# facebookresearch/audiocraft

Hardware: NVIDIA B200
Metric: MusicGen-medium audio-sec/sec @30s gen (higher is better)
Workload: dtype f16

## Files before the change

audiocraft_b200/csrc/lm.cu:

```cuda
#include "common.cuh"
#include "lm_step.cuh"
#include <math.h>
#include <new>
#include <vector>
#include <algorithm>
#include <utility>
#include <stdio.h>
#include <stdlib.h>

__device__ __forceinline__ void mma16816(float (&c)[4], uint32_t a0, uint32_t a1, uint32_t a2, uint32_t a3, uint32_t b0,
                                         uint32_t b1) {
    asm volatile(
        "mma.sync.aligned.m16n8k16.row.col.f32.f16.f16.f32 {%0,%1,%2,%3}, {%4,%5,%6,%7}, {%8,%9}, {%0,%1,%2,%3};"
        : "+f"(c[0]), "+f"(c[1]), "+f"(c[2]), "+f"(c[3])
        : "r"(a0), "r"(a1), "r"(a2), "r"(a3), "r"(b0), "r"(b1));
}

__device__ __forceinline__ void pdl_trigger() { asm volatile("griddepcontrol.launch_dependents;" ::: "memory"); }
__device__ __forceinline__ void pdl_wait() { asm volatile("griddepcontrol.wait;" ::: "memory"); }

#ifdef ACB_TIMELINE
__device__ __forceinline__ void tl_stamp(unsigned long long* t, int slot) {
    if (t && threadIdx.x == 0) {
        unsigned long long now;
// ... 104 lines not shown
    tl_stamp(timing, 5);
    float q = 0.f;
    if (live) {
        const float cx = a.x - mean, cy = a.y - mean, cz = a.z - mean, cw = a.w - mean;
        q = fmaf(cx, cx, q); q = fmaf(cy, cy, q); q = fmaf(cz, cz, q); q = fmaf(cw, cw, q);
    }
    const float rstd = 1.f / sqrtf(block_sum(q, red[1]) / d + 1e-5f);
    tl_stamp(timing, 6);
    if (live) {
        __half2 lo = __floats2half2_rn((a.x - mean) * rstd * gm.x + bt.x, (a.y - mean) * rstd * gm.y + bt.y);
        __half2 hi = __floats2half2_rn((a.z - mean) * rstd * gm.z + bt.z, (a.w - mean) * rstd * gm.w + bt.w);
        uint2 pk;
        pk.x = *reinterpret_cast<uint32_t*>(&lo);
        pk.y = *reinterpret_cast<uint32_t*>(&hi);
        reinterpret_cast<uint2*>(out + (size_t)r * d)[i] = pk;
    }
    tl_stamp(timing, 3);
}

enum { EPI_PARTIAL = 0, EPI_QKV = 1, EPI_GELU = 2, EPI_F32 = 3, EPI_CROSSKV = 4, EPI_QKV_PF = 5 };

struct GemmParams {
    const __half* W;
    const __half* X;
    int N, K, rows, kslice;
    float* out_f32; int ld_out; size_t split_stride;
    __half* out_f16;
    float* q32; __half* kc; __half* vc; int d, H, cache_len; const int* pos;
    int text_len, row0;
    int rows_real;
    unsigned long long* timing;
};

template <int NT, int EPI, int FT2 = 1>
__global__ void __launch_bounds__(128) lm_gemm_kernel(GemmParams p) {
#ifndef ACB_GEMM_U2
#define ACB_GEMM_U2 4
#endif
    constexpr int U = NT <= 2 ? ACB_GEMM_U2 : (NT <= 4 ? 2 : 1);
    constexpr int RP = 8 * NT + 1;
    constexpr int FB = 16 * FT2;
    extern __shared__ __align__(128) unsigned char gsm[];
    const int tid = threadIdx.x, warp = tid >> 5, lane = tid & 31, g = lane >> 2, c4 = lane & 3;
    const int f0 = blockIdx.x * FB;
    const int k0 = blockIdx.y * p.kslice;
    const int ks = min(p.kslice, p.K - k0);
    const int pitch = p.kslice * 2 + 64;
    uint64_t* bar = reinterpret_cast<uint64_t*>(gsm + FB * pitch);
    float* red = reinterpret_cast<float*>(gsm + FB * pitch + 16);

    tl_stamp(p.timing, 0);
    if (tid == 0) mbar_init(bar, 1);
    __syncthreads();
    if (tid == 0) {
        mbar_expect_tx(bar, (uint32_t)FB * (uint32_t)ks * 2u);
#pragma unroll 1
        for (int r = 0; r < FB; ++r)
            bulk_g2s(gsm + r * pitch, p.W + (size_t)(f0 + r) * p.K + k0, (uint32_t)ks * 2u, bar);
    }
    pdl_trigger();
    pdl_wait();
    tl_stamp(p.timing, 1);
    int cache_pos = 0;
    if (EPI == EPI_QKV || EPI == EPI_QKV_PF) cache_pos = p.pos[0];

    float c[FT2][NT][4];
#pragma unroll
    for (int ft = 0; ft < FT2; ++ft)
#pragma unroll
        for (int j = 0; j < NT; ++j) c[ft][j][0] = c[ft][j][1] = c[ft][j][2] = c[ft][j][3] = 0.f;

    const int nkb = ks >> 5;
    const int kbw = (nkb + 3) >> 2;
    const int kb0 = min(nkb, warp * kbw), kb1 = min(nkb, kb0 + kbw);
    const __half* xr = p.X + (size_t)g * p.K + k0 + 8 * c4;
    const unsigned char* wr0 = gsm + g * pitch + 16 * c4;
    const unsigned char* wr1 = wr0 + 8 * pitch;

    bool w_ready = false;
    for (int kb = kb0; kb < kb1; kb += U) {
        uint4 xv[U][NT];
#pragma unroll
        for (int u = 0; u < U; ++u)
#pragma unroll
            for (int j = 0; j < NT; ++j)
                xv[u][j] = (kb + u < kb1) ? *reinterpret_cast<const uint4*>(xr + (size_t)(8 * j) * p.K + (size_t)(kb + u) * 32)
                                          : make_uint4(0, 0, 0, 0);
        if (!w_ready) { mbar_wait(bar, 0); w_ready = true; tl_stamp(p.timing, 4); }
#pragma unroll
        for (int u = 0; u < U; ++u) {
            if (kb + u < kb1) {
#pragma unroll
                for (int ft = 0; ft < FT2; ++ft) {
                    const uint4 wa = *reinterpret_cast<const uint4*>(wr0 + ft * 16 * pitch + (kb + u) * 64);
                    const uint4 wb = *reinterpret_cast<const uint4*>(wr1 + ft * 16 * pitch + (kb + u) * 64);
#pragma unroll
                    for (int j = 0; j < NT; ++j) {
                        mma16816(c[ft][j], wa.x, wb.x, wa.y, wb.y, xv[u][j].x, xv[u][j].y);
                        mma16816(c[ft][j], wa.z, wb.z, wa.w, wb.w, xv[u][j].z, xv[u][j].w);
                    }
                }
            }
        }
    }
    if (!w_ready) mbar_wait(bar, 0);
    tl_stamp(p.timing, 2);
#pragma unroll
    for (int ft = 0; ft < FT2; ++ft)
#pragma unroll
        for (int j = 0; j < NT; ++j) {
            float* r0 = red + (warp * FB + ft * 16 + g) * RP + 8 * j + 2 * c4;
            r0[0] = c[ft][j][0];
            r0[1] = c[ft][j][1];
// ... 184 lines not shown
        }
        __threadfence();
        __syncthreads();
        if (tid == 0) is_last = atomicAdd(p.counter + row * p.H + h, 1) == nact - 1;
        __syncthreads();
        if (is_last) {
            __threadfence();
            if (tid < 64) {
                float M = -INFINITY;
                for (int z = 0; z < nact; ++z) M = fmaxf(M, __ldcg(rec + z * 66));
                float L = 0.f, O = 0.f;
                for (int z = 0; z < nact; ++z) {
                    const float cz = __expf(__ldcg(rec + z * 66) - M);
                    L = fmaf(__ldcg(rec + z * 66 + 1), cz, L);
                    O = fmaf(__ldcg(rec + z * 66 + 2 + tid), cz, O);
                }
                p.out[(size_t)row * p.d + h * 64 + tid] = __float2half_rn(O / L);
            }
            if (tid == 0) p.counter[row * p.H + h] = 0;
        }
    }
    tl_stamp(p.timing, 3);
}

constexpr int ATT2_DEPTH = 8;
__global__ void __launch_bounds__(ATT_WARPS * 32) lm_attn2_kernel(AttnParams p) {
    extern __shared__ __align__(16) unsigned char att2sm[];
    __shared__ float wm[ATT_WARPS], wl[ATT_WARPS], wacc[ATT_WARPS][64];
    const int h = blockIdx.x, tid = threadIdx.x, warp = tid >> 5, lane = tid & 31;
    const int row = blockIdx.y;
    const int sl = lane & 7, pg = lane >> 3;
    tl_stamp(p.timing, 0);
    pdl_trigger();
    pdl_wait();
    tl_stamp(p.timing, 1);
    const int n = p.fixed_len > 0 ? p.fixed_len : p.pos[0] + 1;
    const size_t base = ((size_t)row * p.H + h) * p.cache_len * 64 + sl * 8;
    const __half* kb = p.kc + base;
    const __half* vb = p.vc + base;
    const uint32_t ring = smem_u32(att2sm) + (uint32_t)(warp * ATT2_DEPTH * 1024 + lane * 16);
    const int n_it = (n + 31 - warp * 4) / 32 > 0 ? (n - warp * 4 + 31) / 32 : 0;
    auto issue = [&](int k) {
        if (k < n_it) {
            const int pp = (k * ATT_WARPS + warp) * 4 + pg;
            if (pp < n) {
                const uint32_t d = ring + (uint32_t)((k % ATT2_DEPTH) * 1024);
                asm volatile("cp.async.cg.shared.global [%0], [%1], 16;" ::"r"(d), "l"(kb + (size_t)pp * 64) : "memory");
                asm volatile("cp.async.cg.shared.global [%0], [%1], 16;" ::"r"(d + 512u), "l"(vb + (size_t)pp * 64) : "memory");
            }
        }
        asm volatile("cp.async.commit_group;" ::: "memory");
    };
#pragma unroll
    for (int k = 0; k < ATT2_DEPTH - 1; ++k) issue(k);

    float q[8];
    {
        const float4* qp = reinterpret_cast<const float4*>(p.q + (size_t)row * p.d + h * 64 + sl * 8);
        const float4 qa = qp[0], qb = qp[1];
        q[0] = half_round(qa.x) * p.scale; q[1] = half_round(qa.y) * p.scale; q[2] = half_round(qa.z) * p.scale;
        q[3] = half_round(qa.w) * p.scale; q[4] = half_round(qb.x) * p.scale; q[5] = half_round(qb.y) * p.scale;
        q[6] = half_round(qb.z) * p.scale; q[7] = half_round(qb.w) * p.scale;
    }
    tl_stamp(p.timing, 4);
    OnlineSM st;
    st.m = -INFINITY; st.l = 0.f;
#pragma unroll
    for (int e = 0; e < 8; ++e) st.acc[e] = 0.f;

    for (int k = 0; k < n_it; ++k) {
        issue(k + ATT2_DEPTH - 1);
        asm volatile("cp.async.wait_group %0;" ::"n"(ATT2_DEPTH - 1) : "memory");
        const int pp = (k * ATT_WARPS + warp) * 4 + pg;
        const uint32_t sa = ring + (uint32_t)((k % ATT2_DEPTH) * 1024);
        uint4 kv = make_uint4(0, 0, 0, 0), vv = make_uint4(0, 0, 0, 0);
        if (pp < n) {
            asm volatile("ld.shared.v4.u32 {%0,%1,%2,%3}, [%4];" : "=r"(kv.x), "=r"(kv.y), "=r"(kv.z), "=r"(kv.w) : "r"(sa));
            asm volatile("ld.shared.v4.u32 {%0,%1,%2,%3}, [%4];" : "=r"(vv.x), "=r"(vv.y), "=r"(vv.z), "=r"(vv.w) : "r"(sa + 512u));
        }
        const __half2* k2 = reinterpret_cast<const __half2*>(&kv);
        float s = 0.f;
#pragma unroll
        for (int e = 0; e < 4; ++e) {
            const float2 f = __half22float2(k2[e]);
            s = fmaf(q[2 * e], f.x, s);
            s = fmaf(q[2 * e + 1], f.y, s);
        }
        s += __shfl_xor_sync(0xffffffffu, s, 1);
        s += __shfl_xor_sync(0xffffffffu, s, 2);
        s += __shfl_xor_sync(0xffffffffu, s, 4);
        if (pp < n) {
            const float mn = fmaxf(st.m, s);
            const float corr = __expf(st.m - mn);
            const float pw = __expf(s - mn);
            st.l = st.l * corr + pw;
            const __half2* v2 = reinterpret_cast<const __half2*>(&vv);
#pragma unroll
            for (int e = 0; e < 4; ++e) {
                const float2 f = __half22float2(v2[e]);
                st.acc[2 * e] = fmaf(pw, f.x, st.acc[2 * e] * corr);
                st.acc[2 * e + 1] = fmaf(pw, f.y, st.acc[2 * e + 1] * corr);
            }
            st.m = mn;
        }
// ... 5 lines not shown
        const float m2 = __shfl_xor_sync(0xffffffffu, st.m, o), l2 = __shfl_xor_sync(0xffffffffu, st.l, o);
        float a2[8];
#pragma unroll
        for (int e = 0; e < 8; ++e) a2[e] = __shfl_xor_sync(0xffffffffu, st.acc[e], o);
        osm_merge(st, m2, l2, a2);
    }
    if (pg == 0) {
        if (sl == 0) { wm[warp] = st.m; wl[warp] = st.l; }
#pragma unroll
        for (int e = 0; e < 8; ++e) wacc[warp][sl * 8 + e] = st.acc[e];
    }
    __syncthreads();
    if (tid < 64) {
        float mx = wm[0];
#pragma unroll
        for (int w = 1; w < ATT_WARPS; ++w) mx = fmaxf(mx, wm[w]);
        float l = 0.f, o = 0.f;
#pragma unroll
        for (int w = 0; w < ATT_WARPS; ++w) {
            const float cw = wm[w] == -INFINITY ? 0.f : __expf(wm[w] - mx);
            l = fmaf(wl[w], cw, l);
            o = fmaf(wacc[w][tid], cw, o);
        }
        p.out[(size_t)row * p.d + h * 64 + tid] = __float2half_rn(o / l);
    }
    tl_stamp(p.timing, 3);
}

template <bool PF>
__global__ void __launch_bounds__(256) lm_cross_attn_kernel(AttnParams p, int rows) {
    __shared__ float qs[8][64];
    const int warp = threadIdx.x >> 5, lane = threadIdx.x & 31;
    const int pair = blockIdx.x * 8 + warp;
    tl_stamp(p.timing, 0);
    pdl_trigger();
    pdl_wait();
    tl_stamp(p.timing, 1);
    if (pair >= rows * p.H) return;
    const int row = pair / p.H, h = pair % p.H, n = p.fixed_len;
    {
        const float* qp = p.q + (size_t)row * p.d + h * 64 + lane * 2;
        float2 part[ACB_LM_MAX_SPLIT];
#pragma unroll
        for (int s = 0; s < ACB_LM_MAX_SPLIT; ++s)
            part[s] = s < p.q_nsplit ? *reinterpret_cast<const float2*>(qp + s * p.q_split_stride) : make_float2(0.f, 0.f);
        float a0 = 0.f, a1 = 0.f;
#pragma unroll
        for (int s = 0; s < ACB_LM_MAX_SPLIT; ++s) { a0 += part[s].x; a1 += part[s].y; }
        qs[warp][lane * 2] = half_round(a0) * p.scale;
        qs[warp][lane * 2 + 1] = half_round(a1) * p.scale;
    }
    __syncwarp();
    tl_stamp(p.timing, 4);
    const size_t base = ((size_t)(PF ? row % p.rows_real : row) * p.H + h) * p.cache_len * 64;
    float mx = -INFINITY, l = 0.f, o0 = 0.f, o1 = 0.f;
    for (int t0 = 0; t0 < n; t0 += 32) {
        const int t = t0 + lane;
        float s = -INFINITY;
        if (t < n) {
            const uint4* kr = reinterpret_cast<const uint4*>(p.kc + base + (size_t)t * 64);
            s = 0.f;
#pragma unroll
            for (int c = 0; c < 8; ++c) {
                const uint4 kk = kr[c];
                const __half2* k2 = reinterpret_cast<const __half2*>(&kk);
#pragma unroll
                for (int e = 0; e < 4; ++e) {
                    const float2 f = __half22float2(k2[e]);
                    s = fmaf(qs[warp][c * 8 + 2 * e], f.x, s);
                    s = fmaf(qs[warp][c * 8 + 2 * e + 1], f.y, s);
                }
            }
        }
        tl_stamp(p.timing, 5);
        const float cm = fmaxf(mx, warp_max(s));
        const float corr = mx == -INFINITY ? 0.f : __expf(mx - cm);
        const float pw = t < n ? __expf(s - cm) : 0.f;
        l = l * corr + warp_sum(pw);
        o0 *= corr; o1 *= corr;
        tl_stamp(p.timing, 6);
        const int cnt = min(32, n - t0);
        for (int j = 0; j < cnt; ++j) {
            const float wj = __shfl_sync(0xffffffffu, pw, j);
            const float2 f = __half22float2(*reinterpret_cast<const __half2*>(p.vc + base + (size_t)(t0 + j) * 64 + lane * 2));
            o0 = fmaf(wj, f.x, o0);
            o1 = fmaf(wj, f.y, o1);
        }
        mx = cm;
    }
    tl_stamp(p.timing, 2);
    *reinterpret_cast<__half2*>(p.out + (size_t)row * p.d + h * 64 + lane * 2) = __floats2half2_rn(o0 / l, o1 / l);
    tl_stamp(p.timing, 3);
}

__device__ __forceinline__ uint4 philox4x32_10(uint4 ctr, uint2 key) {
    const uint32_t M0 = 0xD2511F53u, M1 = 0xCD9E8D57u, W0 = 0x9E3779B9u, W1 = 0xBB67AE85u;
#pragma unroll
    for (int r = 0; r < 10; ++r) {
        uint32_t hi0 = __umulhi(M0, ctr.x), lo0 = M0 * ctr.x;
        uint32_t hi1 = __umulhi(M1, ctr.z), lo1 = M1 * ctr.z;
        ctr = make_uint4(hi1 ^ ctr.y ^ key.x, lo1, hi0 ^ ctr.w ^ key.y, lo0);
        key.x += W0;
        key.y += W1;
    }
    return ctr;
}
__device__ __forceinline__ float exp1_noise(uint64_t seed, uint32_t step, uint32_t stream, uint32_t i) {
    uint4 r = philox4x32_10(make_uint4(i >> 2, stream, step, 0x5a17u), make_uint2((uint32_t)seed, (uint32_t)(seed >> 32)));
    uint32_t w = (i & 3) == 0 ? r.x : ((i & 3) == 1 ? r.y : ((i & 3) == 2 ? r.z : r.w));
    float u = ((float)(w >> 8) + 0.5f) * (1.0f / 16777216.0f);
    return -logf(u);
}

struct SampleParams {
    const float* logits;
    const float* noise;
    float* logits_out;
    int64_t* seq; const uint8_t* seq_mask; int* pos; int max_seq;
    int64_t* tokens;
// ... 146 lines not shown
    if (tid == 0) {
        for (int w = 1; w < (nt >> 5); ++w)
            if (bestv[w] > bv || (bestv[w] == bv && besti[w] < bi)) { bv = bestv[w]; bi = besti[w]; }
        if (bi == 0x7fffffff) bi = 0;
        int tok = sorted_space ? si[bi] : bi;
        if (p.tokens) p.tokens[(size_t)b * p.n_q + k] = tok;
        if (p.seq) {
            const int off = cur_pos + 1;
            if (off < p.max_seq) {
                if (!p.seq_mask[(size_t)k * p.max_seq + off]) tok = card;
                int64_t* dst = p.seq + ((size_t)b * p.n_q + k) * p.max_seq + off;
                if (*dst == -1) *dst = tok;
            }
            __threadfence();
            const int done = atomicAdd(p.pos + 1, 1);
            if (done == (int)(gridDim.x * gridDim.y) - 1) { p.pos[1] = 0; p.pos[0] = cur_pos + 1; }
        }
    }
}

__global__ void lm_f32_to_f16_kernel(const float* __restrict__ src, __half* __restrict__ dst, size_t n_valid, size_t n_total) {
    size_t i = (size_t)blockIdx.x * blockDim.x + threadIdx.x;
    if (i < n_total) dst[i] = __float2half_rn(i < n_valid ? src[i] : 0.f);
}

struct acb_lm {
    acb_lm_config cfg;
    acb_lm_weights w;
    acb_lm_buffers buf;
    acb_lm_sampling samp;
    cudaStream_t capture_stream = nullptr;
    cudaGraph_t graph = nullptr;
    cudaGraphExec_t exec = nullptr;
    int batch = 0, rows = 0, rows_pad = 0, text_len = 0, seq_len = 0, sms = 148;
    int launches = 0;
    bool has_cross = false;
    bool pdl = true;
    bool attn2 = true;
    bool fused = false;
    StepLaunch step{};
    unsigned long long* trace = nullptr;
    unsigned long long* timing = nullptr;
    struct TimedGemm { const char* what; int ctas; };
    std::vector<TimedGemm> timed;
};
constexpr int ACB_TIMING_MAX_CTAS = 1024, ACB_TIMING_MAX_GEMMS = 16;
constexpr size_t ACB_PLAN_COUNTER_BYTES = 4096;

template <typename... KArgs, typename... Args>
static cudaError_t launch_k(void (*kernel)(KArgs...), dim3 grid, dim3 block, size_t smem, cudaStream_t s, bool pdl,
                            Args... args) {
    cudaLaunchConfig_t cfg{};
    cfg.gridDim = grid; cfg.blockDim = block; cfg.dynamicSmemBytes = smem; cfg.stream = s;
    cudaLaunchAttribute attr[1];
    if (pdl) {
        attr[0].id = cudaLaunchAttributeProgrammaticStreamSerialization;
        attr[0].val.programmaticStreamSerializationAllowed = 1;
        cfg.attrs = attr; cfg.numAttrs = 1;
    }
    return cudaLaunchKernelEx(&cfg, kernel, KArgs(args)...);
}
#define ACB_LAUNCH(...) ACB_CHECK_CUDA(launch_k(__VA_ARGS__))

static int nt_for_rows(int rows) { return rows <= 8 ? 1 : (rows <= 16 ? 2 : (rows <= 32 ? 4 : 8)); }

static size_t gemm_smem_bytes(int nt, int kslice, int ft2 = 1) {
    return (size_t)16 * ft2 * (kslice * 2 + 64) + 16 + (size_t)4 * 16 * ft2 * (8 * nt + 1) * sizeof(float);
}
constexpr int GEMM_MAX_SMEM = 120 * 1024;

template <int EPI, int FT2>
static int launch_gemm_ft(int nt, const GemmParams& p, int nsplit, cudaStream_t s, bool pdl) {
    dim3 grid(p.N / (16 * FT2), nsplit);
    const size_t smem = gemm_smem_bytes(nt, p.kslice, FT2);
    ACB_REQUIRE(smem <= (size_t)GEMM_MAX_SMEM && p.N % (16 * FT2) == 0, "lm_gemm: tile does not fit (N=%d kslice=%d ft2=%d)", p.N, p.kslice, FT2);
    switch (nt) {
        case 1: ACB_LAUNCH((lm_gemm_kernel<1, EPI, FT2>), grid, dim3(128), smem, s, pdl, p); break;
        case 2: ACB_LAUNCH((lm_gemm_kernel<2, EPI, FT2>), grid, dim3(128), smem, s, pdl, p); break;
        case 4: ACB_LAUNCH((lm_gemm_kernel<4, EPI, FT2>), grid, dim3(128), smem, s, pdl, p); break;
        default: ACB_LAUNCH((lm_gemm_kernel<8, EPI, FT2>), grid, dim3(128), smem, s, pdl, p); break;
    }
    return ACB_OK;
}
template <int EPI>
static int launch_gemm(int nt, const GemmParams& p, int nsplit, cudaStream_t s, bool pdl, int ft2 = 1) {
    if (ft2 == 2) {
        if constexpr (EPI == EPI_CROSSKV || EPI == EPI_QKV_PF) { acb_set_error("lm_gemm: this epilogue uses 16-feature tiles"); return ACB_ERR_INVALID; }
        else return launch_gemm_ft<EPI, 2>(nt, p, nsplit, s, pdl);
    }
    return launch_gemm_ft<EPI, 1>(nt, p, nsplit, s, pdl);
}

template <int NT, int EPI, int FT2>
static cudaError_t gemm_attr_one() {
    cudaError_t e = cudaFuncSetAttribute(lm_gemm_kernel<NT, EPI, FT2>, cudaFuncAttributeMaxDynamicSharedMemorySize, GEMM_MAX_SMEM);
    if (e != cudaSuccess) return e;
    return cudaFuncSetAttribute(lm_gemm_kernel<NT, EPI, FT2>, cudaFuncAttributePreferredSharedMemoryCarveout, 100);
}
template <int EPI>
static cudaError_t gemm_attr_all() {
    cudaError_t e;
    if ((e = gemm_attr_one<1, EPI, 1>()) != cudaSuccess) return e;
    if ((e = gemm_attr_one<2, EPI, 1>()) != cudaSuccess) return e;
    if ((e = gemm_attr_one<4, EPI, 1>()) != cudaSuccess) return e;
    if ((e = gemm_attr_one<8, EPI, 1>()) != cudaSuccess) return e;
    if constexpr (EPI != EPI_CROSSKV && EPI != EPI_QKV_PF) {
        if ((e = gemm_attr_one<1, EPI, 2>()) != cudaSuccess) return e;
        if ((e = gemm_attr_one<2, EPI, 2>()) != cudaSuccess) return e;
        if ((e = gemm_attr_one<4, EPI, 2>()) != cudaSuccess) return e;
        if ((e = gemm_attr_one<8, EPI, 2>()) != cudaSuccess) return e;
    }
    return cudaSuccess;
}

static int pick_ft2(int N, int K, int nsplit, int kslice, int nt, int sms) {
    const char* e = getenv("ACB_LM_FT32");
    const bool enabled = !(e && e[0] == '0');
    if (!enabled || N % 32 != 0 || (size_t)N * K < ((size_t)2 << 20)) return 1;
    if ((N / 32) * nsplit * 10 < sms * 9) return 1;
    if (gemm_smem_bytes(nt, kslice, 2) > (size_t)GEMM_MAX_SMEM) return 1;
    return 2;
}

static int pick_split(int N, int K, int sms, bool allow_split, int* kslice) {
    const int nkb = K / 32, tiles = N / 16;
    int ns = 1;
    if (allow_split) {
        ns = max(acb_ceil_div(K, 1536), acb_ceil_div(2 * sms, tiles));
        ns = max(1, min(min(ns, ACB_LM_MAX_SPLIT), nkb / 2 > 0 ? nkb / 2 : 1));
    }
    int kbs = acb_ceil_div(nkb, ns);
    ns = acb_ceil_div(nkb, kbs);
    *kslice = kbs * 32;
    return ns;
}

static GemmParams base_gemm(const void* W, const void* X, int N, int K, int rows, int kslice) {
    GemmParams p{};
    p.W = (const __half*)W;
    p.X = (const __half*)X;
    p.N = N; p.K = K; p.rows = rows; p.kslice = kslice;
    return p;
}

static int env_int(const char* name, int dflt) {
    const char* e = getenv(name);
    return (e && e[0]) ? atoi(e) : dflt;
}

#define ACB_TRY(expr) do { int rc_ = (expr); if (rc_ != ACB_OK) return rc_; } while (0)

static bool acb_debug_on() {
    static int v = -1;
    if (v < 0) { const char* e = getenv("ACB_DEBUG"); v = (e && e[0] == '1') ? 1 : 0; }
    return v == 1;
}
static int acb_dbg(cudaStream_t s, bool capturing, const char* what, int layer) {
    if (!acb_debug_on() || capturing) return ACB_OK;
    fprintf(stderr, "[acb] %s layer %d ... ", what, layer); fflush(stderr);
    cudaError_t e = cudaStreamSynchronize(s);
    fprintf(stderr, "%s\n", cudaGetErrorString(e)); fflush(stderr);
    if (e != cudaSuccess) { acb_set_error("%s (layer %d): %s", what, layer, cudaGetErrorString(e)); return ACB_ERR_CUDA; }
    return ACB_OK;
}
#define DBG(what, layer) ACB_TRY(acb_dbg(s, capturing, what, layer))

static int enqueue_step_kernels(acb_lm* lm, cudaStream_t s, float* logits_out, int* n_launch, bool gemms_only,
                                bool capturing, int pf_tokens = 0) {
    const acb_lm_config& c = lm->cfg;
    const acb_lm_buffers& B = lm->buf;
    const bool pf = pf_tokens > 0;
    const int rows_real = lm->rows, rows = pf ? rows_real * pf_tokens : rows_real;
    const int d = c.dim, ffn = c.ffn_dim, L = c.num_layers, H = c.num_heads, nt = nt_for_rows(rows);
    const size_t part_stride = (size_t)(pf ? 8 * nt : lm->rows_pad) * d;
    const size_t kv_layer = (size_t)c.max_rows * H * c.max_seq * 64;
    const size_t ckv_layer = (size_t)c.max_rows * H * c.max_text * 64;
    const float scale = 1.0f / sqrtf(64.f);
    const bool pdl = lm->pdl;
    int nl = 0, ks = 0;

    if (!gemms_only) {
        if (pf) ACB_LAUNCH(lm_embed_kernel<true>, dim3(rows), dim3(256), 0, s, pdl, (const __half*)lm->w.emb, lm->w.inv_freq,
                           (const int64_t*)B.seq, (const int*)B.pos, B.x, d, c.n_q, c.card, c.max_seq, lm->batch, c.pos_scale, rows_real);
        else ACB_LAUNCH(lm_embed_kernel<false>, dim3(rows), dim3(256), 0, s, pdl, (const __half*)lm->w.emb, lm->w.inv_freq,
                        (const int64_t*)B.seq, (const int*)B.pos, B.x, d, c.n_q, c.card, c.max_seq, lm->batch, c.pos_scale, rows);
        ++nl;
        DBG("lm_embed_kernel", -1);
    }
    enum { G_QKV, G_O, G_CQ, G_CO, G_FF1, G_FF2, G_HEADS };
    int att_split = env_int("ACB_LM_ATT_SPLIT", 1);
    if (att_split < 1 || att_split > 8 || !B.plan ||
        ACB_PLAN_COUNTER_BYTES + (size_t)rows * H * att_split * 66 * sizeof(float) > ACB_LM_PLAN_BYTES ||
        (size_t)rows * H * sizeof(int) > ACB_PLAN_COUNTER_BYTES)
        att_split = 1;
    if (lm->timing && !capturing) lm->timed.clear();
    auto tl = [&](const char* what, int layer, int ctas) -> unsigned long long* {
        if (!lm->timing || capturing || gemms_only || layer != 0 || (int)lm->timed.size() >= ACB_TIMING_MAX_GEMMS ||
            ctas > ACB_TIMING_MAX_CTAS)
            return nullptr;
        unsigned long long* t = lm->timing + (size_t)lm->timed.size() * ACB_TIMING_MAX_CTAS * 8;
        lm->timed.push_back({what, ctas});
        return t;
    };
    int pending = 0;
    auto ln_launch = [&](const float* gamma, const float* beta, int layer) -> int {
        if (gemms_only) return ACB_OK;
        ACB_LAUNCH(lm_ln_kernel, dim3(rows), dim3(LN_THREADS), 0, s, pdl, B.x, (const float*)B.part, pending, part_stride, gamma, beta,
                   (__half*)B.h16, d, tl("ln", layer, rows));
        ++nl;
        DBG("lm_ln_kernel", layer);
        return ACB_OK;
    };
    auto partial_gemm = [&](const __half* W, const void* X, int N, int K, int layer, int id) -> int {
        const int ns = pick_split(N, K, lm->sms, true, &ks);
        GemmParams p = base_gemm(W, X, N, K, rows, ks);
        p.out_f32 = B.part; p.ld_out = N; p.split_stride = part_stride;
        const int ft2 = pick_ft2(N, K, ns, ks, nt, lm->sms);
        p.timing = tl(id == G_O ? "gemm_O" : (id == G_CQ ? "gemm_CQ" : (id == G_CO ? "gemm_CO" : "gemm_FFN2")), layer, (N / (16 * ft2)) * ns);
        ACB_TRY(launch_gemm<EPI_PARTIAL>(nt, p, ns, s, pdl, ft2));
        ++nl;
        DBG("gemm_EPI_PARTIAL", layer);
        pending = ns;
        return ACB_OK;
    };
    for (int l = 0; l < L; ++l) {
        const float* ln = lm->w.ln + (size_t)l * 6 * d;
        ACB_TRY(ln_launch(ln, ln + d, l));
        {
            pick_split(3 * d, d, lm->sms, false, &ks);
            GemmParams p = base_gemm((const __half*)lm->w.w_qkv + (size_t)l * 3 * d * d, B.h16, 3 * d, d, rows, ks);
            p.q32 = B.q32; p.kc = (__half*)B.k_cache + l * kv_layer; p.vc = (__half*)B.v_cache + l * kv_layer;
            p.d = d; p.H = H; p.cache_len = c.max_seq; p.pos = B.pos; p.rows_real = rows_real;
            const int ft2 = pf ? 1 : pick_ft2(3 * d, d, 1, ks, nt, lm->sms);
            p.timing = tl("gemm_QKV", l, 3 * d / (16 * ft2));
            if (pf) ACB_TRY(launch_gemm<EPI_QKV_PF>(nt, p, 1, s, pdl, 1));
            else ACB_TRY(launch_gemm<EPI_QKV>(nt, p, 1, s, pdl, ft2));
            ++nl;
            DBG("gemm_EPI_QKV", l);
        }
        if (!gemms_only) {
            AttnParams a{B.q32, 1, 0, (__half*)B.k_cache + l * kv_layer, (__half*)B.v_cache + l * kv_layer, (__half*)B.a16,
                         H, d, c.max_seq, B.pos, 0, scale};
            a.timing = tl("attn", l, H * rows * att_split);
            a.part = reinterpret_cast<float*>((unsigned char*)B.plan + ACB_PLAN_COUNTER_BYTES);
            a.counter = reinterpret_cast<int*>(B.plan);
            a.split_min = max(129, env_int("ACB_LM_ATT_SPLIT_MIN", 768));
            a.rows_real = rows_real;
            if (pf) ACB_LAUNCH((lm_attn_kernel<false, true>), dim3(H, rows), dim3(ATT_WARPS * 32), 0, s, pdl, a);
            else if (att_split <= 1 && lm->attn2)
                ACB_LAUNCH(lm_attn2_kernel, dim3(H, rows), dim3(ATT_WARPS * 32), (size_t)ATT_WARPS * ATT2_DEPTH * 1024, s, pdl, a);
            else if (att_split > 1) ACB_LAUNCH(lm_attn_kernel<true>, dim3(H, rows, att_split), dim3(ATT_WARPS * 32), 0, s, pdl, a);
            else ACB_LAUNCH(lm_attn_kernel<false>, dim3(H, rows), dim3(ATT_WARPS * 32), 0, s, pdl, a);
            ++nl;
            DBG("lm_attn_kernel", l);
        }
        ACB_TRY(partial_gemm((const __half*)lm->w.w_o + (size_t)l * d * d, B.a16, d, d, l, G_O));
        if (lm->has_cross) {
            ACB_TRY(ln_launch(ln + 2 * d, ln + 3 * d, l));
            ACB_TRY(partial_gemm((const __half*)lm->w.w_cq + (size_t)l * d * d, B.h16, d, d, l, G_CQ));
            const int nsq = pending;
            pending = 0;
            if (!gemms_only) {
                AttnParams a{B.part, nsq, part_stride, (__half*)B.ck_cache + l * ckv_layer,
                             (__half*)B.cv_cache + l * ckv_layer, (__half*)B.a16, H, d, c.max_text, B.pos, lm->text_len,
                             scale};
                a.timing = tl("cross_attn", l, acb_ceil_div(rows * H, 8));
                a.rows_real = rows_real;
                if (pf) ACB_LAUNCH(lm_cross_attn_kernel<true>, dim3(acb_ceil_div(rows * H, 8)), dim3(256), 0, s, pdl, a, rows);
                else ACB_LAUNCH(lm_cross_attn_kernel<false>, dim3(acb_ceil_div(rows * H, 8)), dim3(256), 0, s, pdl, a, rows);
                ++nl;
                DBG("lm_cross_attn_kernel", l);
            }
            ACB_TRY(partial_gemm((const __half*)lm->w.w_co + (size_t)l * d * d, B.a16, d, d, l, G_CO));
        }
        ACB_TRY(ln_launch(ln + 4 * d, ln + 5 * d, l));
        {
            pick_split(ffn, d, lm->sms, false, &ks);
            GemmParams p = base_gemm((const __half*)lm->w.w_ff1 + (size_t)l * ffn * d, B.h16, ffn, d, rows, ks);
            p.out_f16 = (__half*)B.f16; p.ld_out = ffn;
            const int ft2 = pick_ft2(ffn, d, 1, ks, nt, lm->sms);
            p.timing = tl("gemm_FFN1", l, ffn / (16 * ft2));
            ACB_TRY(launch_gemm<EPI_GELU>(nt, p, 1, s, pdl, ft2)); ++nl;
            DBG("gemm_EPI_GELU", l);
        }
        ACB_TRY(partial_gemm((const __half*)lm->w.w_ff2 + (size_t)l * d * ffn, B.f16, d, ffn, l, G_FF2));
    }
    if (pf) {
        if (n_launch) *n_launch = nl;
        return ACB_OK;
    }
    ACB_TRY(ln_launch(lm->w.out_norm, lm->w.out_norm + d, -1));
    {
        const int N = c.n_q * c.card;
        pick_split(N, d, lm->sms, false, &ks);
        GemmParams p = base_gemm(lm->w.heads, B.h16, N, d, rows, ks);
        p.out_f32 = B.logits; p.ld_out = N;
        ACB_TRY(launch_gemm<EPI_F32>(nt, p, 1, s, pdl, pick_ft2(N, d, 1, ks, nt, lm->sms))); ++nl;
        DBG("gemm_EPI_F32", -1);
    }
    if (!gemms_only) {
        int NP = 1;
        while (NP < c.card) NP <<= 1;
        SampleParams sp{B.logits, lm->samp.noise_from_buffer ? B.noise : nullptr, logits_out, B.seq, B.seq_mask, B.pos,
                        c.max_seq, nullptr, lm->batch, rows, c.n_q, c.card, NP, lm->samp.use_sampling, lm->samp.top_k,
                        lm->samp.temp, lm->samp.top_p, lm->samp.cfg_coef, lm->samp.seed, 0, lm->samp.cfg_coef_beta};
        size_t smem = ((size_t)c.card + 2 * (size_t)NP) * sizeof(float);
        ACB_LAUNCH(lm_sample_kernel, dim3(c.n_q, lm->batch), dim3(1024), smem, s, pdl, sp);
        ++nl;
        DBG("lm_sample_kernel", -1);
    }
    if (n_launch) *n_launch = nl;
    return ACB_OK;
}

static int enqueue_step_fused(acb_lm* lm, cudaStream_t s, float* logits_out, int* n_launch, bool step_only, bool capturing) {
    const acb_lm_config& c = lm->cfg;
    const acb_lm_buffers& B = lm->buf;
    int nl = 0;
    ACB_TRY(lm_step_launch(lm->step, s));
    ++nl;
    DBG("lm_step_kernel", -1);
    if (!step_only) {
        int NP = 1;
        while (NP < c.card) NP <<= 1;
        SampleParams sp{B.logits, lm->samp.noise_from_buffer ? B.noise : nullptr, logits_out, B.seq, B.seq_mask, B.pos,
                        c.max_seq, nullptr, lm->batch, lm->rows, c.n_q, c.card, NP, lm->samp.use_sampling, lm->samp.top_k,
                        lm->samp.temp, lm->samp.top_p, lm->samp.cfg_coef, lm->samp.seed, 0, lm->samp.cfg_coef_beta};
        size_t smem = ((size_t)c.card + 2 * (size_t)NP) * sizeof(float);
        ACB_LAUNCH(lm_sample_kernel, dim3(c.n_q, lm->batch), dim3(1024), smem, s, false, sp);
        ++nl;
        DBG("lm_sample_kernel", -1);
    }
    if (n_launch) *n_launch = nl;
    return ACB_OK;
}

static int enqueue_step(acb_lm* lm, cudaStream_t s, float* logits_out, int* n_launch, bool gemms_only = false,
                        bool capturing = false) {
    if (lm->fused) return enqueue_step_fused(lm, s, logits_out, n_launch, gemms_only, capturing);
    return enqueue_step_kernels(lm, s, logits_out, n_launch, gemms_only, capturing);
}

extern "C" int acb_lm_create(const acb_lm_config* cfg, const acb_lm_weights* w, const acb_lm_buffers* buf, acb_lm_t** out) {
    ACB_REQUIRE(cfg && w && buf && out, "acb_lm_create: null argument");
    ACB_REQUIRE(cfg->dim % 64 == 0 && cfg->dim == cfg->num_heads * 64, "acb_lm_create: head_dim must be 64 (dim=%d heads=%d)",
                cfg->dim, cfg->num_heads);
    ACB_REQUIRE(cfg->dim <= 4 * LN_THREADS, "acb_lm_create: dim %d too large for the LayerNorm kernel", cfg->dim);
    ACB_REQUIRE(cfg->ffn_dim % 32 == 0 && cfg->card % 16 == 0 && cfg->n_q >= 1 && cfg->n_q <= 16, "acb_lm_create: bad ffn/card/n_q");
    ACB_REQUIRE(cfg->card <= 4096, "acb_lm_create: card %d > 4096 not built", cfg->card);
    ACB_REQUIRE(cfg->max_rows >= 1 && cfg->max_rows <= 64, "acb_lm_create: max_rows %d not in [1,64]", cfg->max_rows);
    ACB_REQUIRE(cfg->max_seq >= 2 && cfg->max_seq <= 12000, "acb_lm_create: max_seq %d out of range", cfg->max_seq);
    ACB_REQUIRE(cfg->dim <= 2048, "acb_lm_create: dim %d > 2048: the GEMM stages a 16 x dim weight slab per CTA", cfg->dim);
    acb_lm* lm = new (std::nothrow) acb_lm();
    ACB_REQUIRE(lm, "acb_lm_create: out of host memory");
    lm->cfg = *cfg; lm->w = *w; lm->buf = *buf;
    int dev = 0;
    cudaGetDevice(&dev);
    cudaDeviceGetAttribute(&lm->sms, cudaDevAttrMultiProcessorCount, dev);
    cudaError_t e = cudaStreamCreateWithFlags(&lm->capture_stream, cudaStreamNonBlocking);
    if (e != cudaSuccess) { delete lm; acb_set_error("acb_lm_create: cudaStreamCreate: %s", cudaGetErrorString(e)); return ACB_ERR_CUDA; }
    cudaError_t ea = gemm_attr_all<EPI_PARTIAL>();
    if (ea == cudaSuccess) ea = gemm_attr_all<EPI_QKV>();
    if (ea == cudaSuccess) ea = gemm_attr_all<EPI_GELU>();
    if (ea == cudaSuccess) ea = gemm_attr_all<EPI_F32>();
    if (ea == cudaSuccess) ea = gemm_attr_all<EPI_CROSSKV>();
    if (ea == cudaSuccess) ea = gemm_attr_all<EPI_QKV_PF>();
    if (ea == cudaSuccess) ea = cudaFuncSetAttribute(lm_attn_kernel<false>, cudaFuncAttributePreferredSharedMemoryCarveout, 100);
    if (ea == cudaSuccess) ea = cudaFuncSetAttribute(lm_attn_kernel<true>, cudaFuncAttributePreferredSharedMemoryCarveout, 100);
    if (ea == cudaSuccess) ea = cudaFuncSetAttribute(lm_attn2_kernel, cudaFuncAttributeMaxDynamicSharedMemorySize, ATT_WARPS * ATT2_DEPTH * 1024);
    if (ea == cudaSuccess) ea = cudaFuncSetAttribute(lm_attn2_kernel, cudaFuncAttributePreferredSharedMemoryCarveout, 100);
    if (ea == cudaSuccess) ea = cudaFuncSetAttribute(lm_cross_attn_kernel<false>, cudaFuncAttributePreferredSharedMemoryCarveout, 100);
    if (ea == cudaSuccess) ea = cudaFuncSetAttribute(lm_ln_kernel, cudaFuncAttributePreferredSharedMemoryCarveout, 100);
    if (ea == cudaSuccess) ea = cudaFuncSetAttribute(lm_embed_kernel<false>, cudaFuncAttributePreferredSharedMemoryCarveout, 100);
    if (ea == cudaSuccess) ea = cudaFuncSetAttribute(lm_sample_kernel, cudaFuncAttributePreferredSharedMemoryCarveout, 100);
    if (ea != cudaSuccess) {
        acb_set_error("acb_lm_create: cudaFuncSetAttribute: %s", cudaGetErrorString(ea));
        cudaStreamDestroy(lm->capture_stream);
        delete lm;
        return ACB_ERR_CUDA;
    }
    *out = lm;
    return ACB_OK;
}

static void drop_graph(acb_lm* lm) {
    if (lm->exec) { cudaGraphExecDestroy(lm->exec); lm->exec = nullptr; }
    if (lm->graph) { cudaGraphDestroy(lm->graph); lm->graph = nullptr; }
}

extern "C" int acb_lm_destroy(acb_lm_t* lm) {
    if (!lm) return ACB_OK;
// ... 338 lines not shown
```

Measured before the change: 59.06.

## Stage activations via bulk copies in GEMM and prefetch KV before PDL wait

Adds a STAGED GEMM variant that bulk-copies the activation rows into shared memory with a second mbarrier, replacing per-warp global register loads. A new tiling picker chooses 16/32/48-feature tiles based on a one-wave occupancy estimate using the device's shared memory per SM. The self-attention kernel now issues KV cache prefetches before the PDL wait, skipping the newest position and loading it by hand afterwards. The cross-attention kernel preloads its first K/V chunk into registers before the wait. The embed kernel stops using PDL. Risks include higher shared memory per CTA, which lowers occupancy, and more register pressure in cross-attention.

New measurement: 65.06, median of 6. +10.2%, better.

```diff
diff --git a/audiocraft_b200/csrc/lm.cu b/audiocraft_b200/csrc/lm.cu
--- a/audiocraft_b200/csrc/lm.cu
+++ b/audiocraft_b200/csrc/lm.cu
@@ -160,7 +160,7 @@
     unsigned long long* timing;
 };
 
-template <int NT, int EPI, int FT2 = 1>
+template <int NT, int EPI, int FT2 = 1, bool STAGED = false>
 __global__ void __launch_bounds__(128) lm_gemm_kernel(GemmParams p) {
 #ifndef ACB_GEMM_U2
 #define ACB_GEMM_U2 4
@@ -174,11 +174,15 @@
     const int k0 = blockIdx.y * p.kslice;
     const int ks = min(p.kslice, p.K - k0);
     const int pitch = p.kslice * 2 + 64;
-    uint64_t* bar = reinterpret_cast<uint64_t*>(gsm + FB * pitch);
-    float* red = reinterpret_cast<float*>(gsm + FB * pitch + 16);
+    unsigned char* xs = gsm + FB * pitch;
+    uint64_t* bar = reinterpret_cast<uint64_t*>(xs + (STAGED ? 8 * NT * pitch : 0));
+    float* red = reinterpret_cast<float*>(reinterpret_cast<unsigned char*>(bar) + 16);
 
     tl_stamp(p.timing, 0);
-    if (tid == 0) mbar_init(bar, 1);
+    if (tid == 0) {
+        mbar_init(bar, 1);
+        if (STAGED) mbar_init(bar + 1, 1);
+    }
     __syncthreads();
     if (tid == 0) {
         mbar_expect_tx(bar, (uint32_t)FB * (uint32_t)ks * 2u);
@@ -189,6 +193,13 @@
     pdl_trigger();
     pdl_wait();
     tl_stamp(p.timing, 1);
+    if (STAGED && warp == 0) {
+        if (lane == 0) mbar_expect_tx(bar + 1, 8u * NT * (uint32_t)ks * 2u);
+        __syncwarp();
+#pragma unroll 1
+        for (int r = lane; r < 8 * NT; r += 32)
+            bulk_g2s(xs + r * pitch, p.X + (size_t)r * p.K + k0, (uint32_t)ks * 2u, bar + 1);
+    }
     int cache_pos = 0;
     if (EPI == EPI_QKV || EPI == EPI_QKV_PF) cache_pos = p.pos[0];
 
@@ -206,7 +217,31 @@
     const unsigned char* wr1 = wr0 + 8 * pitch;
 
     bool w_ready = false;
-    for (int kb = kb0; kb < kb1; kb += U) {
+    if (STAGED) {
+        mbar_wait(bar, 0);
+        tl_stamp(p.timing, 4);
+        mbar_wait(bar + 1, 0);
+        tl_stamp(p.timing, 7);
+        w_ready = true;
+        const unsigned char* xg = xs + g * pitch + 16 * c4;
+#pragma unroll 2
+        for (int kb = kb0; kb < kb1; ++kb) {
+            uint4 xv[NT];
+#pragma unroll
+            for (int j = 0; j < NT; ++j) xv[j] = *reinterpret_cast<const uint4*>(xg + 8 * j * pitch + kb * 64);
+#pragma unroll
+            for (int ft = 0; ft < FT2; ++ft) {
+                const uint4 wa = *reinterpret_cast<const uint4*>(wr0 + ft * 16 * pitch + kb * 64);
+                const uint4 wb = *reinterpret_cast<const uint4*>(wr1 + ft * 16 * pitch + kb * 64);
+#pragma unroll
+                for (int j = 0; j < NT; ++j) {
+                    mma16816(c[ft][j], wa.x, wb.x, wa.y, wb.y, xv[j].x, xv[j].y);
+                    mma16816(c[ft][j], wa.z, wb.z, wa.w, wb.w, xv[j].z, xv[j].w);
+                }
+            }
+        }
+    }
+    for (int kb = kb0; !STAGED && kb < kb1; kb += U) {
         uint4 xv[U][NT];
 #pragma unroll
         for (int u = 0; u < U; ++u)
@@ -457,18 +492,16 @@
     const int sl = lane & 7, pg = lane >> 3;
     tl_stamp(p.timing, 0);
     pdl_trigger();
-    pdl_wait();
-    tl_stamp(p.timing, 1);
     const int n = p.fixed_len > 0 ? p.fixed_len : p.pos[0] + 1;
     const size_t base = ((size_t)row * p.H + h) * p.cache_len * 64 + sl * 8;
     const __half* kb = p.kc + base;
     const __half* vb = p.vc + base;
     const uint32_t ring = smem_u32(att2sm) + (uint32_t)(warp * ATT2_DEPTH * 1024 + lane * 16);
     const int n_it = (n + 31 - warp * 4) / 32 > 0 ? (n - warp * 4 + 31) / 32 : 0;
-    auto issue = [&](int k) {
+    auto issue = [&](int k, int lim) {
         if (k < n_it) {
             const int pp = (k * ATT_WARPS + warp) * 4 + pg;
-            if (pp < n) {
+            if (pp < lim) {
                 const uint32_t d = ring + (uint32_t)((k % ATT2_DEPTH) * 1024);
                 asm volatile("cp.async.cg.shared.global [%0], [%1], 16;" ::"r"(d), "l"(kb + (size_t)pp * 64) : "memory");
                 asm volatile("cp.async.cg.shared.global [%0], [%1], 16;" ::"r"(d + 512u), "l"(vb + (size_t)pp * 64) : "memory");
@@ -477,7 +510,16 @@
         asm volatile("cp.async.commit_group;" ::: "memory");
     };
 #pragma unroll
-    for (int k = 0; k < ATT2_DEPTH - 1; ++k) issue(k);
+    for (int k = 0; k < ATT2_DEPTH - 1; ++k) issue(k, n - 1);
+    pdl_wait();
+    tl_stamp(p.timing, 1);
+    const int pl = n - 1, kl = pl >> 5;
+    const bool own_last = kl < ATT2_DEPTH - 1 && ((pl >> 2) & (ATT_WARPS - 1)) == warp && (pl & 3) == pg;
+    uint4 lk = make_uint4(0, 0, 0, 0), lv = lk;
+    if (own_last) {
+        lk = *reinterpret_cast<const uint4*>(kb + (size_t)pl * 64);
+        lv = *reinterpret_cast<const uint4*>(vb + (size_t)pl * 64);
+    }
 
     float q[8];
     {
@@ -487,6 +529,11 @@
         q[3] = half_round(qa.w) * p.scale; q[4] = half_round(qb.x) * p.scale; q[5] = half_round(qb.y) * p.scale;
         q[6] = half_round(qb.z) * p.scale; q[7] = half_round(qb.w) * p.scale;
     }
+    if (own_last) {
+        const uint32_t d = ring + (uint32_t)(kl * 1024);
+        asm volatile("st.shared.v4.u32 [%0], {%1,%2,%3,%4};" ::"r"(d), "r"(lk.x), "r"(lk.y), "r"(lk.z), "r"(lk.w) : "memory");
+        asm volatile("st.shared.v4.u32 [%0], {%1,%2,%3,%4};" ::"r"(d + 512u), "r"(lv.x), "r"(lv.y), "r"(lv.z), "r"(lv.w) : "memory");
+    }
     tl_stamp(p.timing, 4);
     OnlineSM st;
     st.m = -INFINITY; st.l = 0.f;
@@ -494,7 +541,7 @@
     for (int e = 0; e < 8; ++e) st.acc[e] = 0.f;
 
     for (int k = 0; k < n_it; ++k) {
-        issue(k + ATT2_DEPTH - 1);
+        issue(k + ATT2_DEPTH - 1, n);
         asm volatile("cp.async.wait_group %0;" ::"n"(ATT2_DEPTH - 1) : "memory");
         const int pp = (k * ATT_WARPS + warp) * 4 + pg;
         const uint32_t sa = ring + (uint32_t)((k % ATT2_DEPTH) * 1024);
@@ -566,12 +613,27 @@
     __shared__ float qs[8][64];
     const int warp = threadIdx.x >> 5, lane = threadIdx.x & 31;
     const int pair = blockIdx.x * 8 + warp;
+    const bool live = pair < rows * p.H;
+    const int row = pair / p.H, h = pair % p.H, n = p.fixed_len;
+    const size_t base = ((size_t)(PF ? row % p.rows_real : row) * p.H + h) * p.cache_len * 64;
+    uint4 kr[8];
+    __half2 vr[32];
+    auto load_chunk = [&](int t0) {
+        const int t = t0 + lane;
+#pragma unroll
+        for (int c = 0; c < 8; ++c)
+            kr[c] = t < n ? reinterpret_cast<const uint4*>(p.kc + base + (size_t)t * 64)[c] : make_uint4(0, 0, 0, 0);
+#pragma unroll
+        for (int j = 0; j < 32; ++j)
+            vr[j] = t0 + j < n ? *reinterpret_cast<const __half2*>(p.vc + base + (size_t)(t0 + j) * 64 + lane * 2)
+                               : __floats2half2_rn(0.f, 0.f);
+    };
     tl_stamp(p.timing, 0);
+    if (live) load_chunk(0);
     pdl_trigger();
     pdl_wait();
     tl_stamp(p.timing, 1);
-    if (pair >= rows * p.H) return;
-    const int row = pair / p.H, h = pair % p.H, n = p.fixed_len;
+    if (!live) return;
     {
         const float* qp = p.q + (size_t)row * p.d + h * 64 + lane * 2;
         float2 part[ACB_LM_MAX_SPLIT];
@@ -586,18 +648,16 @@
     }
     __syncwarp();
     tl_stamp(p.timing, 4);
-    const size_t base = ((size_t)(PF ? row % p.rows_real : row) * p.H + h) * p.cache_len * 64;
     float mx = -INFINITY, l = 0.f, o0 = 0.f, o1 = 0.f;
     for (int t0 = 0; t0 < n; t0 += 32) {
+        if (t0 > 0) load_chunk(t0);
         const int t = t0 + lane;
         float s = -INFINITY;
         if (t < n) {
-            const uint4* kr = reinterpret_cast<const uint4*>(p.kc + base + (size_t)t * 64);
             s = 0.f;
 #pragma unroll
             for (int c = 0; c < 8; ++c) {
-                const uint4 kk = kr[c];
-                const __half2* k2 = reinterpret_cast<const __half2*>(&kk);
+                const __half2* k2 = reinterpret_cast<const __half2*>(&kr[c]);
 #pragma unroll
                 for (int e = 0; e < 4; ++e) {
                     const float2 f = __half22float2(k2[e]);
@@ -613,12 +673,14 @@
         l = l * corr + warp_sum(pw);
         o0 *= corr; o1 *= corr;
         tl_stamp(p.timing, 6);
-        const int cnt = min(32, n - t0);
-        for (int j = 0; j < cnt; ++j) {
+#pragma unroll
+        for (int j = 0; j < 32; ++j) {
             const float wj = __shfl_sync(0xffffffffu, pw, j);
-            const float2 f = __half22float2(*reinterpret_cast<const __half2*>(p.vc + base + (size_t)(t0 + j) * 64 + lane * 2));
-            o0 = fmaf(wj, f.x, o0);
-            o1 = fmaf(wj, f.y, o1);
+            if (t0 + j < n) {
+                const float2 f = __half22float2(vr[j]);
+                o0 = fmaf(wj, f.x, o0);
+                o1 = fmaf(wj, f.y, o1);
+            }
         }
         mx = cm;
     }
@@ -831,7 +893,7 @@
     cudaStream_t capture_stream = nullptr;
     cudaGraph_t graph = nullptr;
     cudaGraphExec_t exec = nullptr;
-    int batch = 0, rows = 0, rows_pad = 0, text_len = 0, seq_len = 0, sms = 148;
+    int batch = 0, rows = 0, rows_pad = 0, text_len = 0, seq_len = 0, sms = 148, smem_per_sm = 228 * 1024;
     int launches = 0;
     bool has_cross = false;
     bool pdl = true;
@@ -863,62 +925,92 @@
 
 static int nt_for_rows(int rows) { return rows <= 8 ? 1 : (rows <= 16 ? 2 : (rows <= 32 ? 4 : 8)); }
 
-static size_t gemm_smem_bytes(int nt, int kslice, int ft2 = 1) {
-    return (size_t)16 * ft2 * (kslice * 2 + 64) + 16 + (size_t)4 * 16 * ft2 * (8 * nt + 1) * sizeof(float);
-}
-constexpr int GEMM_MAX_SMEM = 120 * 1024;
-
-template <int EPI, int FT2>
+static size_t gemm_smem_bytes(int nt, int kslice, int ft2, bool staged) {
+    const size_t pitch = (size_t)kslice * 2 + 64;
+    return 16 * ft2 * pitch + (staged ? 8 * nt * pitch : 0) + 16 + (size_t)4 * 16 * ft2 * (8 * nt + 1) * sizeof(float);
+}
+constexpr int GEMM_REG_MAX_SMEM = 120 * 1024, GEMM_MAX_SMEM = 227 * 1024;
+
+struct GemmTiling { int ft2; bool staged; };
+
+template <int EPI, int FT2, bool STAGED>
 static int launch_gemm_ft(int nt, const GemmParams& p, int nsplit, cudaStream_t s, bool pdl) {
     dim3 grid(p.N / (16 * FT2), nsplit);
-    const size_t smem = gemm_smem_bytes(nt, p.kslice, FT2);
-    ACB_REQUIRE(smem <= (size_t)GEMM_MAX_SMEM && p.N % (16 * FT2) == 0, "lm_gemm: tile does not fit (N=%d kslice=%d ft2=%d)", p.N, p.kslice, FT2);
+    const size_t smem = gemm_smem_bytes(nt, p.kslice, FT2, STAGED);
+    ACB_REQUIRE(smem <= (size_t)GEMM_MAX_SMEM && p.N % (16 * FT2) == 0, "lm_gemm: tile does not fit (N=%d kslice=%d ft2=%d staged=%d)",
+                p.N, p.kslice, FT2, (int)STAGED);
     switch (nt) {
-        case 1: ACB_LAUNCH((lm_gemm_kernel<1, EPI, FT2>), grid, dim3(128), smem, s, pdl, p); break;
-        case 2: ACB_LAUNCH((lm_gemm_kernel<2, EPI, FT2>), grid, dim3(128), smem, s, pdl, p); break;
-        case 4: ACB_LAUNCH((lm_gemm_kernel<4, EPI, FT2>), grid, dim3(128), smem, s, pdl, p); break;
-        default: ACB_LAUNCH((lm_gemm_kernel<8, EPI, FT2>), grid, dim3(128), smem, s, pdl, p); break;
+        case 1: ACB_LAUNCH((lm_gemm_kernel<1, EPI, FT2, STAGED>), grid, dim3(128), smem, s, pdl, p); break;
+        case 2: ACB_LAUNCH((lm_gemm_kernel<2, EPI, FT2, STAGED>), grid, dim3(128), smem, s, pdl, p); break;
+        case 4: ACB_LAUNCH((lm_gemm_kernel<4, EPI, FT2, STAGED>), grid, dim3(128), smem, s, pdl, p); break;
+        default: ACB_LAUNCH((lm_gemm_kernel<8, EPI, FT2, STAGED>), grid, dim3(128), smem, s, pdl, p); break;
     }
     return ACB_OK;
 }
+constexpr bool gemm_epi_tiled(int epi) { return epi != EPI_CROSSKV && epi != EPI_QKV_PF; }
+
 template <int EPI>
-static int launch_gemm(int nt, const GemmParams& p, int nsplit, cudaStream_t s, bool pdl, int ft2 = 1) {
-    if (ft2 == 2) {
-        if constexpr (EPI == EPI_CROSSKV || EPI == EPI_QKV_PF) { acb_set_error("lm_gemm: this epilogue uses 16-feature tiles"); return ACB_ERR_INVALID; }
-        else return launch_gemm_ft<EPI, 2>(nt, p, nsplit, s, pdl);
-    }
-    return launch_gemm_ft<EPI, 1>(nt, p, nsplit, s, pdl);
-}
-
-template <int NT, int EPI, int FT2>
+static int launch_gemm(int nt, const GemmParams& p, int nsplit, cudaStream_t s, bool pdl, GemmTiling t = {1, false}) {
+    if constexpr (gemm_epi_tiled(EPI)) {
+        if (t.staged) {
+            if (t.ft2 == 3) return launch_gemm_ft<EPI, 3, true>(nt, p, nsplit, s, pdl);
+            if (t.ft2 == 2) return launch_gemm_ft<EPI, 2, true>(nt, p, nsplit, s, pdl);
+            return launch_gemm_ft<EPI, 1, true>(nt, p, nsplit, s, pdl);
+        }
+        if (t.ft2 == 2) return launch_gemm_ft<EPI, 2, false>(nt, p, nsplit, s, pdl);
+    } else if (t.staged || t.ft2 != 1) {
+        acb_set_error("lm_gemm: this epilogue uses 16-feature register-load tiles");
+        return ACB_ERR_INVALID;
+    }
+    return launch_gemm_ft<EPI, 1, false>(nt, p, nsplit, s, pdl);
+}
+
+template <int NT, int EPI, int FT2, bool STAGED>
 static cudaError_t gemm_attr_one() {
-    cudaError_t e = cudaFuncSetAttribute(lm_gemm_kernel<NT, EPI, FT2>, cudaFuncAttributeMaxDynamicSharedMemorySize, GEMM_MAX_SMEM);
+    cudaError_t e = cudaFuncSetAttribute(lm_gemm_kernel<NT, EPI, FT2, STAGED>, cudaFuncAttributeMaxDynamicSharedMemorySize, GEMM_MAX_SMEM);
     if (e != cudaSuccess) return e;
-    return cudaFuncSetAttribute(lm_gemm_kernel<NT, EPI, FT2>, cudaFuncAttributePreferredSharedMemoryCarveout, 100);
+    return cudaFuncSetAttribute(lm_gemm_kernel<NT, EPI, FT2, STAGED>, cudaFuncAttributePreferredSharedMemoryCarveout, 100);
+}
+template <int EPI, int FT2, bool STAGED>
+static cudaError_t gemm_attr_nt() {
+    cudaError_t e;
+    if ((e = gemm_attr_one<1, EPI, FT2, STAGED>()) != cudaSuccess) return e;
+    if ((e = gemm_attr_one<2, EPI, FT2, STAGED>()) != cudaSuccess) return e;
+    if ((e = gemm_attr_one<4, EPI, FT2, STAGED>()) != cudaSuccess) return e;
+    return gemm_attr_one<8, EPI, FT2, STAGED>();
 }
 template <int EPI>
 static cudaError_t gemm_attr_all() {
     cudaError_t e;
-    if ((e = gemm_attr_one<1, EPI, 1>()) != cudaSuccess) return e;
-    if ((e = gemm_attr_one<2, EPI, 1>()) != cudaSuccess) return e;
-    if ((e = gemm_attr_one<4, EPI, 1>()) != cudaSuccess) return e;
-    if ((e = gemm_attr_one<8, EPI, 1>()) != cudaSuccess) return e;
-    if constexpr (EPI != EPI_CROSSKV && EPI != EPI_QKV_PF) {
-        if ((e = gemm_attr_one<1, EPI, 2>()) != cudaSuccess) return e;
-        if ((e = gemm_attr_one<2, EPI, 2>()) != cudaSuccess) return e;
-        if ((e = gemm_attr_one<4, EPI, 2>()) != cudaSuccess) return e;
-        if ((e = gemm_attr_one<8, EPI, 2>()) != cudaSuccess) return e;
+    if ((e = gemm_attr_nt<EPI, 1, false>()) != cudaSuccess) return e;
+    if constexpr (gemm_epi_tiled(EPI)) {
+        if ((e = gemm_attr_nt<EPI, 2, false>()) != cudaSuccess) return e;
+        if ((e = gemm_attr_nt<EPI, 1, true>()) != cudaSuccess) return e;
+        if ((e = gemm_attr_nt<EPI, 2, true>()) != cudaSuccess) return e;
+        if ((e = gemm_attr_nt<EPI, 3, true>()) != cudaSuccess) return e;
     }
     return cudaSuccess;
 }
 
-static int pick_ft2(int N, int K, int nsplit, int kslice, int nt, int sms) {
+static GemmTiling pick_tiling(const acb_lm* lm, int N, int K, int nsplit, int kslice, int nt) {
     const char* e = getenv("ACB_LM_FT32");
-    const bool enabled = !(e && e[0] == '0');
-    if (!enabled || N % 32 != 0 || (size_t)N * K < ((size_t)2 << 20)) return 1;
-    if ((N / 32) * nsplit * 10 < sms * 9) return 1;
-    if (gemm_smem_bytes(nt, kslice, 2) > (size_t)GEMM_MAX_SMEM) return 1;
-    return 2;
+    const bool wide = !(e && e[0] == '0') && (size_t)N * K >= ((size_t)2 << 20);
+    auto one_wave = [&](int ft2, bool staged) {
+        const size_t smem = gemm_smem_bytes(nt, kslice, ft2, staged);
+        if (N % (16 * ft2) != 0 || smem > (size_t)GEMM_MAX_SMEM) return false;
+        const int per_sm = (int)((size_t)lm->smem_per_sm / (smem + 1024));
+        return (N / (16 * ft2)) * nsplit <= lm->sms * per_sm;
+    };
+    if (wide) {
+        for (int ft2 = 2; ft2 <= 3; ++ft2)
+            if (one_wave(ft2, true) && (N / (16 * ft2)) * nsplit * 10 >= lm->sms * 8) return {ft2, true};
+    } else if (one_wave(1, true)) {
+        return {1, true};
+    }
+    if (wide && N % 32 == 0 && (N / 32) * nsplit * 10 >= lm->sms * 9 &&
+        gemm_smem_bytes(nt, kslice, 2, false) <= (size_t)GEMM_REG_MAX_SMEM)
+        return {2, false};
+    return {1, false};
 }
 
 static int pick_split(int N, int K, int sms, bool allow_split, int* kslice) {
@@ -979,9 +1071,9 @@
     int nl = 0, ks = 0;
 
     if (!gemms_only) {
-        if (pf) ACB_LAUNCH(lm_embed_kernel<true>, dim3(rows), dim3(256), 0, s, pdl, (const __half*)lm->w.emb, lm->w.inv_freq,
+        if (pf) ACB_LAUNCH(lm_embed_kernel<true>, dim3(rows), dim3(256), 0, s, false, (const __half*)lm->w.emb, lm->w.inv_freq,
                            (const int64_t*)B.seq, (const int*)B.pos, B.x, d, c.n_q, c.card, c.max_seq, lm->batch, c.pos_scale, rows_real);
-        else ACB_LAUNCH(lm_embed_kernel<false>, dim3(rows), dim3(256), 0, s, pdl, (const __half*)lm->w.emb, lm->w.inv_freq,
+        else ACB_LAUNCH(lm_embed_kernel<false>, dim3(rows), dim3(256), 0, s, false, (const __half*)lm->w.emb, lm->w.inv_freq,
                         (const int64_t*)B.seq, (const int*)B.pos, B.x, d, c.n_q, c.card, c.max_seq, lm->batch, c.pos_scale, rows);
         ++nl;
         DBG("lm_embed_kernel", -1);
@@ -1014,9 +1106,9 @@
         const int ns = pick_split(N, K, lm->sms, true, &ks);
         GemmParams p = base_gemm(W, X, N, K, rows, ks);
         p.out_f32 = B.part; p.ld_out = N; p.split_stride = part_stride;
-        const int ft2 = pick_ft2(N, K, ns, ks, nt, lm->sms);
-        p.timing = tl(id == G_O ? "gemm_O" : (id == G_CQ ? "gemm_CQ" : (id == G_CO ? "gemm_CO" : "gemm_FFN2")), layer, (N / (16 * ft2)) * ns);
-        ACB_TRY(launch_gemm<EPI_PARTIAL>(nt, p, ns, s, pdl, ft2));
+        const GemmTiling t = pick_tiling(lm, N, K, ns, ks, nt);
+        p.timing = tl(id == G_O ? "gemm_O" : (id == G_CQ ? "gemm_CQ" : (id == G_CO ? "gemm_CO" : "gemm_FFN2")), layer, (N / (16 * t.ft2)) * ns);
+        ACB_TRY(launch_gemm<EPI_PARTIAL>(nt, p, ns, s, pdl, t));
         ++nl;
         DBG("gemm_EPI_PARTIAL", layer);
         pending = ns;
@@ -1030,10 +1122,10 @@
             GemmParams p = base_gemm((const __half*)lm->w.w_qkv + (size_t)l * 3 * d * d, B.h16, 3 * d, d, rows, ks);
             p.q32 = B.q32; p.kc = (__half*)B.k_cache + l * kv_layer; p.vc = (__half*)B.v_cache + l * kv_layer;
             p.d = d; p.H = H; p.cache_len = c.max_seq; p.pos = B.pos; p.rows_real = rows_real;
-            const int ft2 = pf ? 1 : pick_ft2(3 * d, d, 1, ks, nt, lm->sms);
-            p.timing = tl("gemm_QKV", l, 3 * d / (16 * ft2));
-            if (pf) ACB_TRY(launch_gemm<EPI_QKV_PF>(nt, p, 1, s, pdl, 1));
-            else ACB_TRY(launch_gemm<EPI_QKV>(nt, p, 1, s, pdl, ft2));
+            const GemmTiling t = pf ? GemmTiling{1, false} : pick_tiling(lm, 3 * d, d, 1, ks, nt);
+            p.timing = tl("gemm_QKV", l, 3 * d / (16 * t.ft2));
+            if (pf) ACB_TRY(launch_gemm<EPI_QKV_PF>(nt, p, 1, s, pdl, t));
+            else ACB_TRY(launch_gemm<EPI_QKV>(nt, p, 1, s, pdl, t));
             ++nl;
             DBG("gemm_EPI_QKV", l);
         }
@@ -1077,9 +1169,9 @@
             pick_split(ffn, d, lm->sms, false, &ks);
             GemmParams p = base_gemm((const __half*)lm->w.w_ff1 + (size_t)l * ffn * d, B.h16, ffn, d, rows, ks);
             p.out_f16 = (__half*)B.f16; p.ld_out = ffn;
-            const int ft2 = pick_ft2(ffn, d, 1, ks, nt, lm->sms);
-            p.timing = tl("gemm_FFN1", l, ffn / (16 * ft2));
-            ACB_TRY(launch_gemm<EPI_GELU>(nt, p, 1, s, pdl, ft2)); ++nl;
+            const GemmTiling t = pick_tiling(lm, ffn, d, 1, ks, nt);
+            p.timing = tl("gemm_FFN1", l, ffn / (16 * t.ft2));
+            ACB_TRY(launch_gemm<EPI_GELU>(nt, p, 1, s, pdl, t)); ++nl;
             DBG("gemm_EPI_GELU", l);
         }
         ACB_TRY(partial_gemm((const __half*)lm->w.w_ff2 + (size_t)l * d * ffn, B.f16, d, ffn, l, G_FF2));
@@ -1094,7 +1186,7 @@
         pick_split(N, d, lm->sms, false, &ks);
         GemmParams p = base_gemm(lm->w.heads, B.h16, N, d, rows, ks);
         p.out_f32 = B.logits; p.ld_out = N;
-        ACB_TRY(launch_gemm<EPI_F32>(nt, p, 1, s, pdl, pick_ft2(N, d, 1, ks, nt, lm->sms))); ++nl;
+        ACB_TRY(launch_gemm<EPI_F32>(nt, p, 1, s, pdl, pick_tiling(lm, N, d, 1, ks, nt))); ++nl;
         DBG("gemm_EPI_F32", -1);
     }
     if (!gemms_only) {
@@ -1156,6 +1248,7 @@
     int dev = 0;
     cudaGetDevice(&dev);
     cudaDeviceGetAttribute(&lm->sms, cudaDevAttrMultiProcessorCount, dev);
+    cudaDeviceGetAttribute(&lm->smem_per_sm, cudaDevAttrMaxSharedMemoryPerMultiprocessor, dev);
     cudaError_t e = cudaStreamCreateWithFlags(&lm->capture_stream, cudaStreamNonBlocking);
     if (e != cudaSuccess) { delete lm; acb_set_error("acb_lm_create: cudaStreamCreate: %s", cudaGetErrorString(e)); return ACB_ERR_CUDA; }
     cudaError_t ea = gemm_attr_all<EPI_PARTIAL>();
```
